# srinix007/GaussianProcessRegression.jl

Hardware: AMD Instinct MI355X
Metric: GP-fit+predict wall-time and K-build GB/s + POTRF TFLOP/s at N=32768 (higher is better)
Workload: dtype f64; 1 GPU; C3 fit+posterior: SE+SE+WN, N=32768, d=8, np=8192; N=32768, d=8, np=8192, kernel=SE+SE+WN, nb=128, parallelism=replicas x1

## Files before the change

### gaussianprocessregression.jl_amd/csrc/common.hpp

```cpp
#pragma once
#include <hip/hip_runtime.h>

#include <cstdio>
#include <string>
#include <vector>

#include "../../include/gpr_hip.h"

#define KMAXP 4

enum { KPROF_SE = 0, KPROF_M32 = 1, KPROF_M52 = 2 };
inline bool kind_stationary(int kind) {
  return kind == GPR_SE || kind == GPR_M32 || kind == GPR_M52 || kind == GPR_PER;
}
inline int kind_hp_width(int kind, int d) {
  return kind == GPR_WN ? 1 : kind == GPR_PER ? 2 * d + 1 : d + 1;
}
inline int kind_profile(int kind) {
  return kind == GPR_M32 ? KPROF_M32 : kind == GPR_M52 ? KPROF_M52 : KPROF_SE;
}
inline const char* kind_name(int kind) {
  return kind == GPR_SE ? "SquaredExp" : kind == GPR_M32 ? "Matern32" : kind == GPR_M52 ? "Matern52"
         : kind == GPR_PER ? "Periodic" : kind == GPR_WN ? "WhiteNoise" : "?";
}

struct KParams {
  int d;
  int nse;
  int has_noise;
  double eps;
  double noise2;
  double noise_sigma;
  double sigma[KMAXP];
  const double* l;
  const double* l2;
  const double* sig;
  const double* pf;
  const double* exptab;
  const int* kinds;
  int nk;
  const double* hp;
  int prof[KMAXP];
  int mix;
  int dx;
  int de;
  int nper;
  const double* per;
  const double* pk;
};

inline KParams kparams_features(const KParams& kp) {
  KParams f = kp;
  f.d = kp.de;
  return f;
}

inline double kp_sigma(const KParams& kp, int p, int* prof = nullptr) {
  int off = 0, se = 0;
  for (int i = 0; i < kp.nk; ++i) {
    if (kp.kinds[i] != GPR_WN) {
      if (se++ == p) {
        if (prof) *prof = kind_profile(kp.kinds[i]);
        return kp.hp[off];
      }
    }
    off += kind_hp_width(kp.kinds[i], kp.dx);
  }
  if (prof) *prof = KPROF_SE;
  return 0.0;
}
inline int kinds_first_non_se(const int* kinds, int nk, int* index) {
  for (int i = 0; i < nk; ++i)
    if (kinds[i] == GPR_M32 || kinds[i] == GPR_M52 || kinds[i] == GPR_PER) {
      if (index) *index = i;
      return kinds[i];
    }
  return 0;
}

inline KParams kparams_group(const KParams& kp, int p0, int cnt, int has_noise) {
  KParams g = kp;
  g.nse = cnt;
  g.has_noise = has_noise;
  g.mix = 0;
  for (int p = 0; p < KMAXP; ++p) {
    g.prof[p] = KPROF_SE;
    g.sigma[p] = p < cnt ? kp_sigma(kp, p0 + p, &g.prof[p]) : 0.0;
    if (g.prof[p] != KPROF_SE) g.mix = 1;
  }
  g.l = kp.l + (size_t)p0 * kp.dx;
  g.l2 = kp.l2 + (size_t)p0 * kp.dx;
  g.sig = kp.sig + p0;
  g.pf = kp.pf + p0;
  if (kp.per) {
    g.per = kp.per + p0;
    g.pk = kp.pk + (size_t)p0 * kp.dx;
  }
  return g;
}

struct KParBlock {
  static constexpr int NSLOT = 8;
  double* dev = nullptr;
  double* host = nullptr;
  size_t cap = 0;
  int next = 0;
  hipEvent_t ev[NSLOT] = {};
  int last = -1;
  size_t last_need = 0;
  int last_nper = 0;
  std::vector<double> tmp;
};

enum TimingClass {
  TC_KBUILD = 0, TC_SYRK = 1, TC_PANEL = 2, TC_TRSM_GEMM = 3, TC_OTHER = 4, TC_GEMM_PIPE = 5,
  TC_DAG = 6, TC_DAG_SOLVE = 7, TC_N = 8
};

struct TimedLaunch {
  int cls;
  hipEvent_t a, b;
  double flops;
};

struct gpr_ctx {
  int device = 0;
  hipStream_t stream = nullptr;
  bool own_stream = false;
  std::string err;
  int nb = 128;
  int nb2 = 1024;
  hipStream_t ls = nullptr;
  hipStream_t stream2 = nullptr;
  hipStream_t srhs = nullptr;
  hipStream_t ssq = nullptr;
  int fused_rhs = -1;
  int fused_rhs_nmax = 16384;
  int fuse_y = 1;
  int fuse_kinv = -1;
  int dag_mode = 1;
  long long dag_spin_limit = 1ll << 25;
  int dag_zlag = 4;
  int dag_lag_built = -1;
  void (*dag_hook)(void* user, const double* dA, int n, int lda, const int* colprog,
                   const int* ustored, int nt, hipEvent_t counters_reset) = nullptr;
  void* dag_hook_user = nullptr;
  int dag_reserve_cu = 0;
  hipEvent_t dag_sync_readers = nullptr;
  bool dag_sync_readers_pending = false;
  bool rhs_solved = false;
  bool gram_full = false;
  int dag_gram = 1;
  int dag_solve = -1;
  int dag_tail = 12288;
  unsigned* dag_tasks = nullptr;
  int dag_ntasks = 0, dag_nt = -1, dag_ntr = -1, dag_flags = -1;
  int* dag_sync = nullptr;
  size_t dag_sync_cap = 0;
  double* dpadA = nullptr;
  size_t padA_cap = 0;
  double* dpadB = nullptr;
  size_t padB_cap = 0;
  void* rb_handle = nullptr;
  int (*rb_destroy)(void*) = nullptr;
  int ncu = 0;
  std::vector<hipEvent_t> sync_events;
  size_t ev_next = 0;

  double* winv = nullptr;
  size_t winv_cap = 0;
  const double* fac_ptr = nullptr;
  int fac_n = 0, fac_ld = 0, fac_nb = 0;
  bool fac_valid = false;

  int* dinfo = nullptr;
  double* dexptab = nullptr;
  double* dscratch = nullptr;
  size_t scratch_cap = 0;
  static constexpr int CV_MAX_SUB = 8;
  struct gpr_ctx* cv_sub[CV_MAX_SUB] = {};
  int cv_streams = 4;
  double* dbig = nullptr;
  size_t big_cap = 0;
  double* dbig2 = nullptr;
  size_t big2_cap = 0;
  double* dsqinv = nullptr;
  size_t sqinv_cap = 0;
  int sqinv_nb2 = 0;
  const double* sq_ptr = nullptr;
  int sq_n = 0, sq_ld = 0;
  double* dpanel = nullptr;
  size_t panel_cap = 0;
  double* dtrsv = nullptr;
  size_t trsv_cap = 0;
  double* dxs = nullptr;
  size_t xs_cap = 0;
  double* dxps = nullptr;
  size_t xps_cap = 0;
  double* dscr_wt = nullptr;
  size_t scr_wt_cap = 0;
  double* dpanel_rhs = nullptr;
  size_t panel_rhs_cap = 0;
  double* dgA = nullptr;
  size_t gA_cap = 0;
  double* dgB = nullptr;
  size_t gB_cap = 0;
  double* dgc = nullptr;
  size_t gc_cap = 0;
  struct KupList {
    long long key = -1;
    int nitems = 0;
    int* d = nullptr;
    unsigned long long used = 0;
  };
  KupList kup[4];
  unsigned long long kup_clock = 0;
  const double* kup_ptr = nullptr;
  int kup_n = 0, kup_ld = 0;
  double* dagb = nullptr;
  size_t dagb_cap = 0;
  double* deig = nullptr;
  size_t eig_cap = 0;
  double* ddc = nullptr;
  size_t dc_cap = 0;
  int* dc_tab_host = nullptr;
  size_t dc_tab_host_cap = 0;
  hipEvent_t dc_tab_ev = nullptr;
  double* dtri = nullptr;
  size_t tri_cap = 0;
  int kbuild_upper = 1;
  int kbuild_exact = 0;
  int kbuild_gram_maxd = 1 << 30;
  KParBlock kpar;
  int kbuild_tiles = 0;
  int kbuild_colstore = 1;
  int cv_batch = 1;
  double cv_batch_gb = 16.0;
  double quad_batch_gb = 16.0;
  int quad_eigen = -1;
  int quad_seq = 0;

  bool timing = false;
  std::vector<TimedLaunch> pending;
  std::vector<hipEvent_t> event_pool;
  double t_ms[TC_N] = {};
  long long t_launches[TC_N] = {};
  double t_flops[TC_N] = {};
};

int split_predict_pieces(gpr_ctx* ctx, const int* kinds, int nk, const double* hp, int d,
                         const double* dX, int ns, const double* dU, int ldu, const double* dwt,
                         const double* dXe, int ne, const double* dXq, int nq, const int* pieces,
                         int npieces, int var_lo, int var_hi, double eps, double* dmu, int ldmu,
                         double* dvar, bool compact);
int set_err(gpr_ctx* ctx, int code, const char* fmt, ...);
void copy_knobs(const gpr_ctx* from, gpr_ctx* to);

#define HIP_TRY(ctx, expr)                                                          \
  do {                                                                              \
    hipError_t _e = (expr);                                                         \
    if (_e != hipSuccess)                                                           \
      return set_err(ctx, GPR_E_HIP, "%s failed: %s (%s:%d)", #expr,                \
                     hipGetErrorString(_e), __FILE__, __LINE__);                    \
  } while (0)

#define GPR_TRY(expr)            \
  do {                           \
    int _r = (expr);             \
    if (_r != 0) return _r;      \
  } while (0)

#define LAUNCH_CHECK(ctx) HIP_TRY(ctx, hipGetLastError())

inline int refuse_non_se(gpr_ctx* ctx, const int* kinds, int nk, const char* what) {
  int idx = 0;
  const int kind = kinds ? kinds_first_non_se(kinds, nk, &idx) : 0;
  if (!kind) return 0;
  return set_err(ctx, GPR_E_UNSUP, "%s needs SquaredExp parts: part %d is %s", what, idx + 1,
                 kind_name(kind));
}

int ensure_buf(gpr_ctx* ctx, double** p, size_t* cap, size_t need_doubles);
int ensure_winv(gpr_ctx* ctx, int n, int nb);

struct TimerScope {
  gpr_ctx* ctx;
  TimedLaunch tl;
  bool on;
  hipStream_t st;
  TimerScope(gpr_ctx* c, int cls, double flops);
  ~TimerScope();
};

int make_kparams(gpr_ctx* ctx, const int* kinds, int nk, const double* hp, int d,
                 double eps, KParams* kp, int* D_total);

// ... 71 lines not shown
```

### gaussianprocessregression.jl_amd/csrc/dag.hip

```cpp
#include <algorithm>
#include <cstdint>
#include <type_traits>

#include "common.hpp"

#ifdef DAG_TRACE
__device__ unsigned long long g_diag_ph[16];
#define DSTAMP_INIT() unsigned long long _dst_t = __builtin_amdgcn_s_memrealtime()
#define DSTAMP(i)                                                   \
  do {                                                              \
    __syncthreads();                                                \
    if (threadIdx.x == 0) {                                         \
      const unsigned long long _t = __builtin_amdgcn_s_memrealtime(); \
      atomicAdd(&g_diag_ph[i], _t - _dst_t);                        \
      if ((i) == 7) atomicAdd(&g_diag_ph[8], 1ull);                 \
      _dst_t = _t;                                                  \
    }                                                               \
  } while (0)
#define DSTAMPW(i)                                                  \
  do {                                                              \
    const unsigned long long _t = __builtin_amdgcn_s_memrealtime(); \
    if (threadIdx.x == 0) atomicAdd(&g_diag_ph[i], _t - _dst_t);    \
    _dst_t = _t;                                                    \
  } while (0)
// ... 441 lines not shown
#pragma unroll
      for (int ii = 0; ii < 4; ++ii)
#pragma unroll
        for (int r = 0; r < 4; ++r) {
          const int nn = wn * 64 + ii * 16 + (lane >> 4) + 4 * r;
          const double* col = T + (size_t)min(nn, nv - 1) * ldt;
#pragma unroll
          for (int jj = 0; jj < 4; ++jj) {
            const int mm = wm * 64 + jj * 16 + (lane & 15);
            const double c = col[min(mm, mv - 1)];
            acc[ii][jj][r] = (mm < mv && nn < nv) ? -c : 0.0;
          }
        }
      if (a.mirror && !rhs && !diag) {
        double* Tm = a.A + (size_t)j * DT + (size_t)i * DT * a.lda;
#pragma unroll
        for (int ii = 0; ii < 4; ++ii)
#pragma unroll
          for (int jj = 0; jj < 4; ++jj)
#pragma unroll
            for (int r = 0; r < 4; ++r) {
              const int nn = wn * 64 + ii * 16 + (lane >> 4) + 4 * r;
              const int mm = wm * 64 + jj * 16 + (lane & 15);
              if (mm < mv && nn < nv) Tm[(size_t)nn + (size_t)mm * a.lda] = -acc[ii][jj][r];
            }
      }
      DTRACE(1, 2);
      int done = (rhs && a.lower) ? j : 0;
      while (done < i) {
        int r = 0;
        PROF(p_wait, r = dag_wait(colprog + i, pj, done, i, a.info, a.spin_limit, &s_wait));
        PROF(p_acc, dag_accum(acc, Pcol + (size_t)done * DT, a.lda, mv, Qcol + (size_t)done * DT,
                              ldt, nv, (r - done) * (DT / DTK), lds));
        done = r;
      }
      if (diag) {
        double* S = lds;
#pragma unroll
        for (int ii = 0; ii < 4; ++ii)
#pragma unroll
          for (int r = 0; r < 4; ++r) {
            const int nn = wn * 64 + ii * 16 + (lane >> 4) + 4 * r;
#pragma unroll
            for (int jj = 0; jj < 4; ++jj) {
              const int mm = wm * 64 + jj * 16 + (lane & 15);
              if (mm <= nn) S[pk(mm, nn)] = nn < mv ? -acc[ii][jj][r] : (mm == nn ? 1.0 : 0.0);
            }
          }
        __syncthreads();
        DTRACE(1, 3);
        int f = 0;
        PROF(p_fac, f = dag_factor(S, mv, a.kglob + i * DT, a.winv + (size_t)i * DT * DT));
        if (f && w == 0) atomicCAS(a.info, 0, f);
        s_fok = f == 0;
        DTRACE(1, 4);
      } else {
        if (i > 0) {
#pragma unroll
          for (int ii = 0; ii < 4; ++ii)
#pragma unroll
            for (int r = 0; r < 4; ++r) {
              const int nn = wn * 64 + ii * 16 + (lane >> 4) + 4 * r;
#pragma unroll
              for (int jj = 0; jj < 4; ++jj) {
                const int mm = wm * 64 + jj * 16 + (lane & 15);
                if (mm < mv && nn < nv) T[(size_t)mm + (size_t)nn * ldt] = -acc[ii][jj][r];
              }
            }
        }
        asm volatile("s_waitcnt vmcnt(0)" ::: "memory");
        __builtin_amdgcn_fence(__ATOMIC_RELEASE, "workgroup");
        PROF(p_wait, dag_wait(colprog + i, colprog + i, i, i + 1, a.info, a.spin_limit, &s_wait));
#pragma unroll
        for (int ii = 0; ii < 4; ++ii)
#pragma unroll
          for (int jj = 0; jj < 4; ++jj) acc[ii][jj] = d4v{0.0, 0.0, 0.0, 0.0};
        const bool tri = mv == DT;
        if (tri)
          PROF(p_tri, dag_accum<true>(acc, a.winv + (size_t)i * DT * DT, DT, mv, T, ldt, nv, DT / DTK, lds));
        else
          PROF(p_tri, dag_accum(acc, a.winv + (size_t)i * DT * DT, DT, mv, T, ldt, nv, mv / DTK, lds));
#pragma unroll
        for (int ii = 0; ii < 4; ++ii)
#pragma unroll
          for (int r = 0; r < 4; ++r) {
            const int nn = wn * 64 + ii * 16 + (lane >> 4) + 4 * r;
#pragma unroll
            for (int jj = 0; jj < 4; ++jj) {
              const int mm = (tri ? 16 * dag_mblk(wm, jj) : wm * 64 + jj * 16) + (lane & 15);
              if (mm < mv && nn < nv) st_res<true>(&T[(size_t)mm + (size_t)nn * ldt], acc[ii][jj][r]);
            }
          }
      }
    } else if (a.mirror && !rhs && !diag) {
      double* Tm = a.A + (size_t)j * DT + (size_t)i * DT * a.lda;
      for (int e = tid; e < DT * DT; e += 256) {
        const int mm = e & (DT - 1), nn = e >> 7;
        if (mm < mv && nn < nv) Tm[(size_t)nn + (size_t)mm * a.lda] = T[(size_t)mm + (size_t)nn * ldt];
      }
    }
    DTRACE(1, 5);
#ifdef DAG_PROF_PUB
    if (diag) PROF(p_pub, dag_publish(pj, i + 1)); else dag_publish(pj, i + 1);
#else
    dag_publish(pj, i + 1);
#endif
    DTRACE(1, 6);
    if (diag && !skip && __builtin_amdgcn_readfirstlane(s_fok))
      dag_store_u(lds, T, a.lda, mv, a.ustored != nullptr);
    if (diag && a.ustored) dag_publish(a.ustored + i, 1);
    ++p_n;
  }
  DTRACE(1, 7);
#ifdef DAG_TRACE
  p_all = __builtin_amdgcn_s_memrealtime() - p_start;
  DTRACE(2, (int)p_wait);
  DTRACE(3, (int)p_acc);
  DTRACE(4, (int)p_fac);
#ifdef DAG_PROF_PUB
#undef p_tri
  DTRACE(5, (int)p_pub);
  (void)p_tri_unused;
#else
  DTRACE(5, (int)p_tri);
#endif
  DTRACE(6, (int)p_all);
  DTRACE(7, (int)p_n);
#endif
}

}

__global__ void dag_init_kernel(int* sync, int nt, int ntr, int solve, int lower) {
  for (int t = blockIdx.x * blockDim.x + threadIdx.x; t < nt + ntr; t += gridDim.x * blockDim.x)
    sync[2 + t] = t < nt ? (solve ? t + 1 : 0) : (lower ? t - nt : 0);
}

static long long dag_spin_limit(const gpr_ctx* ctx) {
#ifdef GPR_TESTING
  if (const char* sl = getenv("GPR_DAG_SPIN_LIMIT")) return std::max(1ll, atoll(sl));
#endif
  return ctx->dag_spin_limit;
}

bool dag_shape_ok(int n, int lda, const double* dA) {
  return n > 0 && n % 16 == 0 && lda % 16 == 0 && lda <= DAG_LD_MAX && ((uintptr_t)dA & 127) == 0 &&
         n <= DT * 32767;
}

extern "C" int gpr_debug_dag_shape_ok(int n, int lda, unsigned long long addr) {
  return dag_shape_ok(n, lda, reinterpret_cast<const double*>((uintptr_t)addr)) ? 1 : 0;
}

bool dag_takes_whole(const gpr_ctx* ctx, int n, int lda, const double* dA) {
  (void)lda;
  (void)dA;
  return ctx->dag_mode && ctx->nb == DT && n > 0 &&
         n <= DT * 32767 - 16;
}

__global__ void dag_pad_in_kernel(const double* __restrict__ A, size_t lda, int n,
                                  double* __restrict__ W, int n2) {
  const size_t tot = (size_t)n2 * n2;
  for (size_t t = blockIdx.x * (size_t)blockDim.x + threadIdx.x; t < tot;
       t += (size_t)gridDim.x * blockDim.x) {
    const int r = (int)(t % n2), c = (int)(t / n2);
    if (r <= c) W[t] = c < n ? A[(size_t)r + (size_t)c * lda] : (r == c ? 1.0 : 0.0);
  }
}

__global__ void dag_pad_out_kernel(double* __restrict__ A, size_t lda, int n,
                                   const double* __restrict__ W, int n2) {
  const size_t tot = (size_t)n * n;
  for (size_t t = blockIdx.x * (size_t)blockDim.x + threadIdx.x; t < tot;
       t += (size_t)gridDim.x * blockDim.x) {
    const int r = (int)(t % n), c = (int)(t / n);
    if (r <= c) A[(size_t)r + (size_t)c * lda] = W[(size_t)r + (size_t)c * n2];
  }
}

int launch_potrf_dag_padded(gpr_ctx* ctx, double* dA, int n, int lda, double* dB, int nrhs,
                            int ldb) {
  const int n2 = (n + 15) / 16 * 16;
  hipStream_t st = ctx->stream;
  if (ensure_buf(ctx, &ctx->dpadA, &ctx->padA_cap, (size_t)n2 * n2) != 0 ||
      (dB && ensure_buf(ctx, &ctx->dpadB, &ctx->padB_cap, (size_t)n2 * nrhs) != 0)) {
    ctx->err.clear();
    (void)hipGetLastError();
    return 1;
  }
  const int blocks = 2048;
  dag_pad_in_kernel<<<blocks, 256, 0, st>>>(dA, (size_t)lda, n, ctx->dpadA, n2);
  LAUNCH_CHECK(ctx);
  if (dB) {
    HIP_TRY(ctx, hipMemcpy2DAsync(ctx->dpadB, (size_t)n2 * sizeof(double), dB,
                                  (size_t)ldb * sizeof(double), (size_t)n * sizeof(double), nrhs,
                                  hipMemcpyDeviceToDevice, st));
    if (n2 > n)
      HIP_TRY(ctx, hipMemset2DAsync(ctx->dpadB + n, (size_t)n2 * sizeof(double), 0,
                                    (size_t)(n2 - n) * sizeof(double), nrhs, st));
  }
  const int rc = launch_potrf_dag(ctx, ctx->dpadA, n2, n2, dB ? ctx->dpadB : nullptr, nrhs, n2, 0,
                                  st, 0);
  if (rc) return rc < 0 ? rc : set_err(ctx, GPR_E_HIP, "padded tile-DAG: shape not eligible");
  dag_pad_out_kernel<<<blocks, 256, 0, st>>>(dA, (size_t)lda, n, ctx->dpadA, n2);
  LAUNCH_CHECK(ctx);
  if (dB)
    HIP_TRY(ctx, hipMemcpy2DAsync(dB, (size_t)ldb * sizeof(double), ctx->dpadB,
                                  (size_t)n2 * sizeof(double), (size_t)n * sizeof(double), nrhs,
                                  hipMemcpyDeviceToDevice, st));
  return 0;
}

int launch_potrf_dag(gpr_ctx* ctx, double* dA, int n, int lda, double* dB, int nrhs, int ldb,
                     int kglob, hipStream_t st, int flags, double* dG, int ldg) {
  const bool solve = flags & DAG_SOLVE, lower = flags & DAG_LOWER, gram = flags & DAG_GRAM;
  const bool mirror = flags & DAG_MIRROR;
  if ((solve || lower) && (!dB || kglob)) return 1;
  if (mirror && (solve || kglob)) return 1;
  if (gram && (!lower || !dG || ldg < n || nrhs != n)) return 1;
  if (ctx->nb != DT || n <= 0 || n % 16 || lda % 16 || lda > DAG_LD_MAX || ((uintptr_t)dA & 127) ||
      n > DT * 32767 || kglob % DT)
    return 1;
  if (dB && (nrhs <= 0 || ldb % 16 || ldb > DAG_LD_MAX || ((uintptr_t)dB & 127) || nrhs > DT * 65535))
    return 1;
  const int nt = (n + DT - 1) / DT, ntr = dB ? (nrhs + DT - 1) / DT : 0;
  GPR_TRY(ensure_winv(ctx, kglob + n, DT));
  if (ctx->dag_nt != nt || ctx->dag_ntr != ntr || ctx->dag_flags != (flags & ~DAG_MIRROR) ||
      ctx->dag_lag_built != ctx->dag_zlag) {
    std::vector<unsigned> tasks;
    tasks.reserve((size_t)nt * (nt + 1) + (size_t)nt * ntr);
    const int lag = solve || !lower ? 0 : std::min(ctx->dag_zlag, nt);
    auto rhs_row = [&](int i) {
      for (int c = 0; c < (lower ? std::min(ntr, i + 1) : ntr); ++c)
        tasks.push_back(0x80000000u | ((unsigned)i << 16) | (unsigned)c);
    };
    for (int i = 0; i < nt; ++i) {
      if (!solve)
        for (int j = i; j < nt; ++j) tasks.push_back(((unsigned)i << 16) | (unsigned)j);
      if (i - lag >= 0) rhs_row(i - lag);
    }
    for (int i = std::max(nt - lag, 0); i < nt; ++i) rhs_row(i);
    if (gram)
      for (int j = 0; j < nt; ++j)
        for (int i = 0; i <= j; ++i) tasks.push_back(((unsigned)i << 16) | (unsigned)j);
    if (ctx->dag_tasks) {
      HIP_TRY(ctx, hipStreamSynchronize(ctx->stream));
      HIP_TRY(ctx, hipFree(ctx->dag_tasks));
    }
    ctx->dag_tasks = nullptr;
    ctx->dag_nt = ctx->dag_ntr = -1;
    HIP_TRY(ctx, hipMalloc((void**)&ctx->dag_tasks, tasks.size() * sizeof(unsigned)));
    HIP_TRY(ctx, hipMemcpy(ctx->dag_tasks, tasks.data(), tasks.size() * sizeof(unsigned),
                           hipMemcpyHostToDevice));
    ctx->dag_ntasks = (int)tasks.size();
    ctx->dag_nt = nt;
    ctx->dag_ntr = ntr;
    ctx->dag_flags = flags & ~DAG_MIRROR;
    ctx->dag_lag_built = ctx->dag_zlag;
  }
  if (ctx->dag_sync_readers_pending) {
    HIP_TRY(ctx, hipStreamWaitEvent(st, ctx->dag_sync_readers, 0));
    HIP_TRY(ctx, hipStreamWaitEvent(ctx->stream, ctx->dag_sync_readers, 0));
    ctx->dag_sync_readers_pending = false;
  }
  const size_t nsync = 2 + (size_t)nt + ntr + nt;
  if (ctx->dag_sync_cap < nsync) {
    if (ctx->dag_sync) {
      HIP_TRY(ctx, hipStreamSynchronize(ctx->stream));
      HIP_TRY(ctx, hipFree(ctx->dag_sync));
    }
    ctx->dag_sync = nullptr;
    ctx->dag_sync_cap = 0;
    HIP_TRY(ctx, hipMalloc((void**)&ctx->dag_sync, nsync * sizeof(int)));
    ctx->dag_sync_cap = nsync;
  }
  HIP_TRY(ctx, hipMemsetAsync(ctx->dag_sync, 0, nsync * sizeof(int), st));
  if (solve || lower) {
    dag_init_kernel<<<(nt + ntr + 255) / 256, 256, 0, st>>>(ctx->dag_sync, nt, ntr, solve, lower);
    LAUNCH_CHECK(ctx);
  }
  if (ctx->ncu <= 0) {
    hipDeviceProp_t prop;
    HIP_TRY(ctx, hipGetDeviceProperties(&prop, ctx->device));
    ctx->ncu = prop.multiProcessorCount;
  }
  DagArgs a{};
  a.A = dA;
  a.lda = (size_t)lda;
  a.n = n;
  a.nt = nt;
  a.B = dB;
  a.ldb = (size_t)(dB ? ldb : 0);
  a.nrhs = dB ? nrhs : 0;
  a.ntr = ntr;
  a.winv = ctx->winv + (size_t)(kglob / DT) * DT * DT;
  a.kglob = kglob;
  a.info = ctx->dinfo;
  a.sync = ctx->dag_sync;
  a.tasks = ctx->dag_tasks;
  a.ntasks = ctx->dag_ntasks;
  a.lower = lower;
  a.G = gram ? dG : nullptr;
  a.ldg = (size_t)(gram ? ldg : 0);
  a.gbase = gram ? ctx->dag_ntasks - nt * (nt + 1) / 2 : ctx->dag_ntasks;
  a.mirror = mirror;
  a.spin_limit = dag_spin_limit(ctx);
  const int grid = std::min(ctx->dag_ntasks, std::max(1, ctx->ncu - ctx->dag_reserve_cu));
  auto hook = (ctx->dag_hook && !solve && !lower && kglob == 0) ? ctx->dag_hook : nullptr;
  a.ustored = hook ? ctx->dag_sync + 2 + nt + ntr : nullptr;
  hipEvent_t hook_ev = nullptr;
  if (hook) {
    ctx->dag_hook = nullptr;
    if (hipEventCreateWithFlags(&hook_ev, hipEventDisableTiming) != hipSuccess) hook_ev = nullptr;
    if (hook_ev && hipEventRecord(hook_ev, st) != hipSuccess) {
      hipEventDestroy(hook_ev);
      hook_ev = nullptr;
    }
    (void)hipGetLastError();
  }
  const double flops = (solve ? 0.0 : (double)n * n * n / 3.0) +
                       (lower ? (double)n * n * n / 3.0 : (double)n * n * (dB ? nrhs : 0)) +
                       (gram ? (double)n * n * n / 3.0 : 0.0);
  {
    hipStream_t ls = ctx->ls;
    ctx->ls = st;
    TimerScope ts(ctx, solve ? TC_DAG_SOLVE : TC_DAG, flops);
    if (gram)
      potrf_dag_kernel<true, false><<<grid, 256, 0, st>>>(a);
    else
      potrf_dag_kernel<false, false><<<grid, 256, 0, st>>>(a);
    ctx->ls = ls;
    const hipError_t le = hipGetLastError();
    if (le != hipSuccess) {
      if (hook_ev) hipEventDestroy(hook_ev);
      return set_err(ctx, GPR_E_HIP, "tile-DAG launch: %s", hipGetErrorString(le));
    }
  }
  if (hook) {
    hook(ctx->dag_hook_user, dA, n, lda, ctx->dag_sync + 2, a.ustored, nt, hook_ev);
    if (hook_ev) hipEventDestroy(hook_ev);
  }
  return 0;
}

int launch_potrf_dag_batch(gpr_ctx* ctx, double* dA, size_t strA, int n, int lda, double* dB,
                           size_t strB, int nrhs, int ldb, int nbatch, int* info_out) {
  hipStream_t st = ctx->stream;
  if (nbatch <= 0) return 0;
  if (n <= 0 || n % 16 || lda % 16 || lda > DAG_LD_MAX || strA % 16 || ((uintptr_t)dA & 127) ||
      n > DT * 32767)
    return 1;
  if (dB && (nrhs <= 0 || ldb % 16 || ldb > DAG_LD_MAX || strB % 16 || ((uintptr_t)dB & 127) ||
             nrhs > DT * 65535))
    return 1;
  const int nt = (n + DT - 1) / DT, ntr = dB ? (nrhs + DT - 1) / DT : 0;
  std::vector<unsigned> tasks;
  std::vector<int> tb;
  const size_t per = (size_t)nt * (nt + 1) / 2 + (size_t)nt * ntr;
  tasks.reserve(per * nbatch);
  tb.reserve(per * nbatch);
  for (int i = 0; i < nt; ++i) {
    for (int b = 0; b < nbatch; ++b)
      for (int j = i; j < nt; ++j) {
        tasks.push_back(((unsigned)i << 16) | (unsigned)j);
        tb.push_back(b);
      }
    for (int b = 0; b < nbatch; ++b)
      for (int c = 0; c < ntr; ++c) {
        tasks.push_back(0x80000000u | ((unsigned)i << 16) | (unsigned)c);
        tb.push_back(b);
      }
  }
  const int ntasks = (int)tasks.size();
  const int strS = 2 + nt + ntr;
  const size_t nW = (size_t)nbatch * nt * DT * DT;
  const size_t nI = (size_t)ntasks * 2 + (size_t)nbatch * strS + (size_t)nbatch;
  GPR_TRY(ensure_buf(ctx, &ctx->dagb, &ctx->dagb_cap, nW + (nI + 1) / 2 + 1));
  double* W = ctx->dagb;
  unsigned* dtasks = reinterpret_cast<unsigned*>(W + nW);
  int* dtb = reinterpret_cast<int*>(dtasks + ntasks);
  int* dsync = dtb + ntasks;
  int* dinfo = dsync + (size_t)nbatch * strS;
  HIP_TRY(ctx, hipMemcpyAsync(dtasks, tasks.data(), sizeof(unsigned) * ntasks, hipMemcpyHostToDevice, st));
  HIP_TRY(ctx, hipMemcpyAsync(dtb, tb.data(), sizeof(int) * ntasks, hipMemcpyHostToDevice, st));
  HIP_TRY(ctx, hipMemsetAsync(dsync, 0, sizeof(int) * ((size_t)nbatch * strS + nbatch), st));
  if (ctx->ncu <= 0) {
    hipDeviceProp_t prop;
    HIP_TRY(ctx, hipGetDeviceProperties(&prop, ctx->device));
    ctx->ncu = prop.multiProcessorCount;
  }
  DagArgs a{};
  a.A = dA;
  a.lda = (size_t)lda;
  a.n = n;
  a.nt = nt;
  a.B = dB;
  a.ldb = (size_t)(dB ? ldb : 0);
  a.nrhs = dB ? nrhs : 0;
  a.ntr = ntr;
  a.winv = W;
  a.kglob = 0;
  a.info = dinfo;
  a.sync = dsync;
  a.tasks = dtasks;
  a.ntasks = ntasks;
  a.gbase = ntasks;
  a.spin_limit = dag_spin_limit(ctx);
  a.tbatch = dtb;
  a.strA = strA;
  a.strB = strB;
  a.strW = (size_t)nt * DT * DT;
// ... 19 lines not shown
```

### gaussianprocessregression.jl_amd/csrc/gpr_ctx.hip

```cpp
#include <algorithm>
#include <cmath>
#include <cstdarg>
#include <cstdlib>
#include <cstring>

#include "common.hpp"

int set_err(gpr_ctx* ctx, int code, const char* fmt, ...) {
  if (ctx) {
    char buf[1024];
    va_list ap;
    va_start(ap, fmt);
    vsnprintf(buf, sizeof buf, fmt, ap);
    va_end(ap);
    ctx->err = buf;
  }
  return code;
}

int ensure_buf(gpr_ctx* ctx, double** p, size_t* cap, size_t need) {
  if (*cap >= need && *p) return 0;
  if (*p) {
    HIP_TRY(ctx, hipStreamSynchronize(ctx->stream));
    HIP_TRY(ctx, hipFree(*p));
// ... 38 lines not shown
TimerScope::~TimerScope() {
  if (!on) return;
  hipEventRecord(tl.b, st);
  ctx->pending.push_back(tl);
}

static void drain_timing(gpr_ctx* ctx) {
  if (ctx->pending.empty()) return;
  hipStreamSynchronize(ctx->stream);
  for (auto& t : ctx->pending) {
    float ms = 0;
    hipEventElapsedTime(&ms, t.a, t.b);
    ctx->t_ms[t.cls] += ms;
    ctx->t_launches[t.cls] += 1;
    ctx->t_flops[t.cls] += t.flops;
    ctx->event_pool.push_back(t.a);
    ctx->event_pool.push_back(t.b);
  }
  ctx->pending.clear();
}

int make_kparams(gpr_ctx* ctx, const int* kinds, int nk, const double* hp, int d, double eps,
                 KParams* kp, int* D_total) {
  if (!kinds || nk <= 0) return set_err(ctx, GPR_E_ARG, "bad kinds/nk (%d)", nk);
  if (!hp) return set_err(ctx, GPR_E_ARG, "hp is NULL");
  if (d <= 0) return set_err(ctx, GPR_E_ARG, "d=%d (needs d >= 1)", d);
  memset(kp, 0, sizeof *kp);
  int nse = 0, nper = 0;
  for (int i = 0, off = 0; i < nk; ++i) {
    if (kind_stationary(kinds[i])) ++nse;
    else if (kinds[i] != GPR_WN) return set_err(ctx, GPR_E_ARG, "unknown kernel kind %d", kinds[i]);
    if (kinds[i] == GPR_PER) {
      ++nper;
      for (int k = 0; k < d; ++k) {
        const double p = hp[off + 1 + d + k];
        if (!(std::fabs(p) > 0.0) || std::isinf(p))
          return set_err(ctx, GPR_E_ARG, "part %d (Periodic): period p_%d = %g of dimension %d is "
                                         "zero or not finite", i + 1, k + 1, p, k + 1);
      }
    }
    off += kind_hp_width(kinds[i], d);
  }
  if (nse == 0)
    return set_err(ctx, GPR_E_ARG, "kernel needs at least one stationary part (SquaredExp, "
                                   "Matern32, Matern52 or Periodic)");
  KParBlock& kb = ctx->kpar;
  const size_t nl = (size_t)nse * d;
  const size_t need = 2 * nl + 2 * (size_t)nse + (nper ? nl + (size_t)nse : 0);
  if (need > kb.cap || !kb.dev) {
    const size_t cap = std::max(need, (size_t)(2 * 4 * 64 + 2 * 4));
    if (kb.dev) {
      HIP_TRY(ctx, hipStreamSynchronize(ctx->stream));
      HIP_TRY(ctx, hipFree(kb.dev));
      HIP_TRY(ctx, hipHostFree(kb.host));
      kb.dev = kb.host = nullptr;
      kb.cap = 0;
    }
    const size_t bytes = KParBlock::NSLOT * cap * sizeof(double);
    if (hipMalloc((void**)&kb.dev, bytes) != hipSuccess) {
      kb.dev = nullptr;
      return set_err(ctx, GPR_E_NOMEM, "hipMalloc of %zu bytes failed", bytes);
    }
    if (hipHostMalloc((void**)&kb.host, bytes, hipHostMallocDefault) != hipSuccess) {
      hipFree(kb.dev);
      kb.dev = kb.host = nullptr;
      return set_err(ctx, GPR_E_NOMEM, "hipHostMalloc of %zu bytes failed", bytes);
    }
    kb.cap = cap;
    kb.last = -1;
  }
  kb.tmp.resize(need);
  double* hl = kb.tmp.data();
  kp->exptab = ctx->dexptab;
  kp->d = kp->dx = d;
  kp->de = nper ? 2 * d : d;
  kp->nper = nper;
  kp->eps = eps;
  kp->kinds = kinds;
  kp->nk = nk;
  kp->hp = hp;
  int off = 0;
  for (int i = 0; i < nk; ++i) {
    if (kinds[i] != GPR_WN) {
      const int prof = kind_profile(kinds[i]);
      if (kp->nse < KMAXP) {
        kp->sigma[kp->nse] = hp[off];
        kp->prof[kp->nse] = prof;
      }
      if (prof != KPROF_SE) kp->mix = 1;
      hl[2 * nl + kp->nse] = hp[off];
      hl[2 * nl + nse + kp->nse] = (double)prof;
      for (int k = 0; k < d; ++k) {
        hl[(size_t)kp->nse * d + k] = hp[off + 1 + k];
        hl[nl + (size_t)kp->nse * d + k] = hp[off + 1 + k] * hp[off + 1 + k];
      }
      if (nper) {
        const bool per = kinds[i] == GPR_PER;
        hl[2 * nl + 2 * nse + kp->nse] = per ? 1.0 : 0.0;
        for (int k = 0; k < d; ++k)
          hl[2 * nl + 3 * (size_t)nse + (size_t)kp->nse * d + k] = per ? hp[off + 1 + d + k] : 1.0;
      }
      kp->nse++;
      off += kind_hp_width(kinds[i], d);
    } else {
      if (!kp->has_noise) {
        kp->has_noise = 1;
        kp->noise_sigma = hp[off];
        kp->noise2 = hp[off] * hp[off];
      }
      off += 1;
    }
  }
  int slot = kb.last;
  if (slot < 0 || kb.last_need != need || kb.last_nper != nper ||
      memcmp(kb.host + (size_t)slot * kb.cap, hl, need * sizeof(double)) != 0) {
    slot = kb.next;
    kb.next = (slot + 1) % KParBlock::NSLOT;
    if (!kb.ev[slot]) HIP_TRY(ctx, hipEventCreateWithFlags(&kb.ev[slot], hipEventDisableTiming));
    else HIP_TRY(ctx, hipEventSynchronize(kb.ev[slot]));
    kb.last = -1;
    memcpy(kb.host + (size_t)slot * kb.cap, hl, need * sizeof(double));
    HIP_TRY(ctx, hipMemcpyAsync(kb.dev + (size_t)slot * kb.cap, kb.host + (size_t)slot * kb.cap,
                                need * sizeof(double), hipMemcpyHostToDevice, ctx->stream));
    HIP_TRY(ctx, hipEventRecord(kb.ev[slot], ctx->stream));
    kb.last = slot;
    kb.last_need = need;
    kb.last_nper = nper;
  }
  const double* dl = kb.dev + (size_t)slot * kb.cap;
  kp->l = dl;
  kp->l2 = dl + nl;
  kp->sig = dl + 2 * nl;
  kp->pf = dl + 2 * nl + nse;
  if (nper) {
    kp->per = dl + 2 * nl + 2 * nse;
    kp->pk = dl + 2 * nl + 3 * (size_t)nse;
  }
  if (D_total) *D_total = off;
  return 0;
}

namespace {
struct Knob {
  const char* name;
  int gpr_ctx::*ip;
  double gpr_ctx::*dp;
};
const Knob kKnobs[] = {
    {"GPR_DAG", &gpr_ctx::dag_mode, nullptr},
    {"GPR_DAG_TAIL", &gpr_ctx::dag_tail, nullptr},
    {"GPR_DAG_SOLVE", &gpr_ctx::dag_solve, nullptr},
    {"GPR_DAG_GRAM", &gpr_ctx::dag_gram, nullptr},
    {"GPR_DAG_ZLAG", &gpr_ctx::dag_zlag, nullptr},
    {"GPR_FUSED_RHS", &gpr_ctx::fused_rhs, nullptr},
    {"GPR_FUSE_Y", &gpr_ctx::fuse_y, nullptr},
    {"GPR_FUSE_KINV", &gpr_ctx::fuse_kinv, nullptr},
    {"GPR_KBUILD_UPPER", &gpr_ctx::kbuild_upper, nullptr},
    {"GPR_KBUILD_EXACT", &gpr_ctx::kbuild_exact, nullptr},
    {"GPR_KBUILD_COLSTORE", &gpr_ctx::kbuild_colstore, nullptr},
    {"GPR_KBUILD_TILES", &gpr_ctx::kbuild_tiles, nullptr},
    {"GPR_KBUILD_GRAM_MAXD", &gpr_ctx::kbuild_gram_maxd, nullptr},
    {"GPR_CV_STREAMS", &gpr_ctx::cv_streams, nullptr},
    {"GPR_CV_BATCH", &gpr_ctx::cv_batch, nullptr},
    {"GPR_CV_BATCH_GB", nullptr, &gpr_ctx::cv_batch_gb},
    {"GPR_QUAD_BATCH_GB", nullptr, &gpr_ctx::quad_batch_gb},
    {"GPR_QUAD_EIGEN", &gpr_ctx::quad_eigen, nullptr},
    {"GPR_QUAD_SEQ", &gpr_ctx::quad_seq, nullptr},
};

void knob_set(gpr_ctx* ctx, const Knob& k, double v) {
  if (k.ip) {
    int iv = (int)v;
    if (k.ip == &gpr_ctx::dag_zlag) iv = std::max(0, iv);
    if (k.ip == &gpr_ctx::cv_streams) iv = std::max(1, std::min(iv, (int)gpr_ctx::CV_MAX_SUB));
    ctx->*k.ip = iv;
  } else {
    ctx->*k.dp = v;
  }
}

const Knob* knob_find(const char* name) {
  if (!name) return nullptr;
  for (const Knob& k : kKnobs)
    if (!strcmp(k.name, name)) return &k;
  return nullptr;
}
}

void copy_knobs(const gpr_ctx* from, gpr_ctx* to) {
  for (const Knob& k : kKnobs) {
    if (k.ip) to->*k.ip = from->*k.ip;
    else to->*k.dp = from->*k.dp;
  }
  to->dag_spin_limit = from->dag_spin_limit;
}

extern "C" {

const char* gpr_version(void) { return "gpr_hip 0.1.0 (gfx950)"; }

int gpr_ctx_create(int device, void* stream, gpr_ctx_t* out) {
  if (!out) return GPR_E_ARG;
  *out = nullptr;
  gpr_ctx* ctx = new gpr_ctx();
  ctx->device = device;
  if (hipSetDevice(device) != hipSuccess) {
    delete ctx;
    return GPR_E_HIP;
  }
  if (stream) {
    ctx->stream = (hipStream_t)stream;
  } else {
    if (hipStreamCreateWithFlags(&ctx->stream, hipStreamNonBlocking) != hipSuccess) {
      delete ctx;
      return GPR_E_HIP;
    }
    ctx->own_stream = true;
  }
  ctx->ls = ctx->stream;
  int prio_lo = 0, prio_hi = 0;
  hipDeviceGetStreamPriorityRange(&prio_lo, &prio_hi);
  if (hipStreamCreateWithPriority(&ctx->stream2, hipStreamNonBlocking, prio_hi) != hipSuccess ||
      hipStreamCreateWithFlags(&ctx->srhs, hipStreamNonBlocking) != hipSuccess ||
      hipStreamCreateWithFlags(&ctx->ssq, hipStreamNonBlocking) != hipSuccess) {
    delete ctx;
    return GPR_E_HIP;
  }
  if (const char* e = getenv("GPU_MAX_HW_QUEUES")) {
    const int q = atoi(e);
    if (q > 0) ctx->cv_streams = std::min(ctx->cv_streams, q);
  }
  for (const Knob& k : kKnobs)
    if (const char* e = getenv(k.name)) knob_set(ctx, k, atof(e));
  if (hipMalloc((void**)&ctx->dinfo, 64) != hipSuccess) {
    delete ctx;
    return GPR_E_NOMEM;
  }
  {
    double tab[256];
    for (int j = 0; j < 256; ++j) tab[j] = (double)exp2l((long double)j / 256.0L);
    if (hipMalloc((void**)&ctx->dexptab, sizeof tab) != hipSuccess ||
        hipMemcpy(ctx->dexptab, tab, sizeof tab, hipMemcpyHostToDevice) != hipSuccess) {
      hipFree(ctx->dinfo);
      delete ctx;
      return GPR_E_NOMEM;
    }
  }
  *out = ctx;
  return 0;
}

int gpr_ctx_destroy(gpr_ctx_t ctx) {
  if (!ctx) return 0;
  for (auto* sub : ctx->cv_sub) gpr_ctx_destroy(sub);
  hipStreamSynchronize(ctx->stream);
  if (ctx->dag_sync_readers) {
    hipEventSynchronize(ctx->dag_sync_readers);
    hipEventDestroy(ctx->dag_sync_readers);
  }
  drain_timing(ctx);
  for (auto e : ctx->event_pool) hipEventDestroy(e);
  for (auto e : ctx->sync_events) hipEventDestroy(e);
  if (ctx->stream2) hipStreamDestroy(ctx->stream2);
  if (ctx->srhs) hipStreamDestroy(ctx->srhs);
  if (ctx->ssq) hipStreamDestroy(ctx->ssq);
  if (ctx->dpanel_rhs) hipFree(ctx->dpanel_rhs);
  if (ctx->dscr_wt) hipFree(ctx->dscr_wt);
  if (ctx->dag_tasks) hipFree(ctx->dag_tasks);
  if (ctx->dag_sync) hipFree(ctx->dag_sync);
  if (ctx->dpadA) hipFree(ctx->dpadA);
  if (ctx->dpadB) hipFree(ctx->dpadB);
  if (ctx->rb_handle && ctx->rb_destroy) ctx->rb_destroy(ctx->rb_handle);
  if (ctx->winv) hipFree(ctx->winv);
  if (ctx->dinfo) hipFree(ctx->dinfo);
  if (ctx->dexptab) hipFree(ctx->dexptab);
  if (ctx->dscratch) hipFree(ctx->dscratch);
  if (ctx->dbig) hipFree(ctx->dbig);
  if (ctx->dbig2) hipFree(ctx->dbig2);
  if (ctx->dtrsv) hipFree(ctx->dtrsv);
  if (ctx->dsqinv) hipFree(ctx->dsqinv);
  if (ctx->dpanel) hipFree(ctx->dpanel);
  if (ctx->dxs) hipFree(ctx->dxs);
  if (ctx->dxps) hipFree(ctx->dxps);
  if (ctx->dgA) hipFree(ctx->dgA);
  if (ctx->dgB) hipFree(ctx->dgB);
  if (ctx->dgc) hipFree(ctx->dgc);
  if (ctx->kpar.dev) hipFree(ctx->kpar.dev);
  if (ctx->kpar.host) hipHostFree(ctx->kpar.host);
  for (auto e : ctx->kpar.ev)
    if (e) hipEventDestroy(e);
  for (auto& e : ctx->kup)
    if (e.d) hipFree(e.d);
  if (ctx->deig) hipFree(ctx->deig);
  if (ctx->ddc) hipFree(ctx->ddc);
  if (ctx->dc_tab_ev) hipEventDestroy(ctx->dc_tab_ev);
  if (ctx->dc_tab_host) hipHostFree(ctx->dc_tab_host);
  if (ctx->dtri) hipFree(ctx->dtri);
  if (ctx->dagb) hipFree(ctx->dagb);
  if (ctx->own_stream) hipStreamDestroy(ctx->stream);
  delete ctx;
  return 0;
}

const char* gpr_last_error(gpr_ctx_t ctx) { return ctx ? ctx->err.c_str() : "null context"; }

int gpr_sync(gpr_ctx_t ctx) {
  HIP_TRY(ctx, hipStreamSynchronize(ctx->stream));
  return 0;
}

void* gpr_ctx_stream(gpr_ctx_t ctx) { return ctx ? (void*)ctx->stream : nullptr; }

int gpr_malloc(gpr_ctx_t ctx, size_t bytes, void** dptr) {
  if (!dptr) return set_err(ctx, GPR_E_ARG, "dptr is NULL");
  if (hipMalloc(dptr, bytes ? bytes : 1) != hipSuccess)
    return set_err(ctx, GPR_E_NOMEM, "hipMalloc(%zu) failed", bytes);
  return 0;
}

int gpr_free(gpr_ctx_t ctx, void* dptr) {
  HIP_TRY(ctx, hipStreamSynchronize(ctx->stream));
  if (dptr) HIP_TRY(ctx, hipFree(dptr));
  return 0;
}

int gpr_upload(gpr_ctx_t ctx, void* dst, const void* src, size_t bytes) {
  HIP_TRY(ctx, hipMemcpyAsync(dst, src, bytes, hipMemcpyHostToDevice, ctx->stream));
  HIP_TRY(ctx, hipStreamSynchronize(ctx->stream));
  return 0;
}

int gpr_download(gpr_ctx_t ctx, void* dst, const void* src, size_t bytes) {
  HIP_TRY(ctx, hipMemcpyAsync(dst, src, bytes, hipMemcpyDeviceToHost, ctx->stream));
  HIP_TRY(ctx, hipStreamSynchronize(ctx->stream));
  return 0;
}

int gpr_set_block(gpr_ctx_t ctx, int nb) {
  if (nb != 64 && nb != 128) return set_err(ctx, GPR_E_ARG, "nb must be 64 or 128 (got %d)", nb);
  ctx->nb = nb;
  if (ctx->nb2 % nb) ctx->nb2 = 4 * nb;
  ctx->fac_valid = false;
  return 0;
}

int gpr_set_outer_block(gpr_ctx_t ctx, int nb2) {
  if (nb2 < ctx->nb || nb2 % ctx->nb)
    return set_err(ctx, GPR_E_ARG, "outer block %d must be a multiple of nb=%d", nb2, ctx->nb);
  ctx->nb2 = nb2;
  return 0;
}

int gpr_set_knob(gpr_ctx_t ctx, const char* name, double value) {
  if (!ctx) return GPR_E_ARG;
  const Knob* k = knob_find(name);
  if (!k) return set_err(ctx, GPR_E_ARG, "unknown knob %s", name ? name : "(null)");
  knob_set(ctx, *k, value);
  if (k->ip == &gpr_ctx::dag_zlag) ctx->dag_lag_built = -1;
  return 0;
}

int gpr_get_knob(gpr_ctx_t ctx, const char* name, double* value) {
  if (!ctx || !value) return GPR_E_ARG;
  const Knob* k = knob_find(name);
  if (!k) return set_err(ctx, GPR_E_ARG, "unknown knob %s", name ? name : "(null)");
  *value = k->ip ? (double)(ctx->*k->ip) : ctx->*k->dp;
  return 0;
}

int gpr_forget_factor(gpr_ctx_t ctx) {
  ctx->fac_valid = false;
  ctx->fac_ptr = nullptr;
  ctx->sqinv_nb2 = 0;
  ctx->sq_ptr = nullptr;
  return 0;
}

int gpr_timing_enable(gpr_ctx_t ctx, int on) {
  ctx->timing = on != 0;
  return 0;
}

int gpr_timing_get(gpr_ctx_t ctx, int cls, double* ms, long long* launches, double* flops) {
  if (cls < 0 || cls >= TC_N) return set_err(ctx, GPR_E_ARG, "bad timing class %d", cls);
  drain_timing(ctx);
  if (ms) *ms = ctx->t_ms[cls];
  if (launches) *launches = ctx->t_launches[cls];
  if (flops) *flops = ctx->t_flops[cls];
  return 0;
}

int gpr_timing_reset(gpr_ctx_t ctx) {
  drain_timing(ctx);
  for (int i = 0; i < TC_N; ++i) {
    ctx->t_ms[i] = 0;
    ctx->t_launches[i] = 0;
    ctx->t_flops[i] = 0;
  }
  return 0;
}

}
```

Before: 3.380 GP jobs/s (fit N=32768 + posterior mean/var np=8192, per GPU).

## Interleave DAG task order across row groups after a leading panel

Adds a configurable task ordering for the persistent DAG Cholesky/solve scheduler. For non-lower, non-gram runs, rows past a threshold (default 32) are emitted in groups of up to 4 and interleaved column by column, optionally with a skew between rows. The aim is to expose more concurrent ready tasks and reduce stalls waiting on dependencies late in the factorization. The interleaving can also delay the critical-path panel tasks. Knobs and a debug export are added, and the rebuild key now covers the new parameters.

```diff
diff --git a/gaussianprocessregression.jl_amd/csrc/common.hpp b/gaussianprocessregression.jl_amd/csrc/common.hpp
--- a/gaussianprocessregression.jl_amd/csrc/common.hpp
+++ b/gaussianprocessregression.jl_amd/csrc/common.hpp
@@ -141,7 +141,8 @@
   int dag_mode = 1;
   long long dag_spin_limit = 1ll << 25;
   int dag_zlag = 4;
-  int dag_lag_built = -1;
+  int dag_rgroup = 4, dag_rskew = 0, dag_rgroup_min = 32;
+  int dag_order_built[4] = {-1, -1, -1, -1};
   void (*dag_hook)(void* user, const double* dA, int n, int lda, const int* colprog,
                    const int* ustored, int nt, hipEvent_t counters_reset) = nullptr;
   void* dag_hook_user = nullptr;
diff --git a/gaussianprocessregression.jl_amd/csrc/dag.hip b/gaussianprocessregression.jl_amd/csrc/dag.hip
--- a/gaussianprocessregression.jl_amd/csrc/dag.hip
+++ b/gaussianprocessregression.jl_amd/csrc/dag.hip
@@ -617,6 +617,56 @@
   return dag_shape_ok(n, lda, reinterpret_cast<const double*>((uintptr_t)addr)) ? 1 : 0;
 }
 
+std::vector<unsigned> dag_task_order(int nt, int ntr, bool solve, bool lower, bool gram, int zlag,
+                                     int group, int skew, int gmin) {
+  std::vector<unsigned> tasks;
+  tasks.reserve((size_t)nt * (nt + 1) + (size_t)nt * ntr);
+  const int lag = solve || !lower ? 0 : std::min(std::max(zlag, 0), nt);
+  auto a_task = [&](int i, int j) { tasks.push_back(((unsigned)i << 16) | (unsigned)j); };
+  auto rhs_task = [&](int i, int c) {
+    tasks.push_back(0x80000000u | ((unsigned)i << 16) | (unsigned)c);
+  };
+  auto rhs_row = [&](int i) {
+    for (int c = 0; c < (lower ? std::min(ntr, i + 1) : ntr); ++c) rhs_task(i, c);
+  };
+  const int R = (lower || gram || group < 2) ? 1 : (group < 4 ? 2 : 4);
+  const int g0 = R == 1 ? nt : (int)std::min<long long>(nt, ((long long)std::max(gmin, 0) + R - 1) / R * R);
+  const int sk = std::min(std::max(skew, 0), std::max(nt, ntr));
+  for (int i = 0; i < g0; ++i) {
+    if (!solve)
+      for (int j = i; j < nt; ++j) a_task(i, j);
+    if (i - lag >= 0) rhs_row(i - lag);
+  }
+  for (int i = std::max(nt - lag, 0); i < nt; ++i) rhs_row(i);
+  for (int g = g0; g < nt; g += R) {
+    const int m = std::min(R, nt - g);
+    if (!solve)
+      for (int s = 0; s < nt - g + (m - 1) * sk; ++s)
+        for (int r = 0; r < m; ++r) {
+          const int j = g + s - r * sk;
+          if (j >= g + r && j < nt) a_task(g + r, j);
+        }
+    for (int s = 0; s < ntr + (m - 1) * sk; ++s)
+      for (int r = 0; r < m; ++r) {
+        const int c = s - r * sk;
+        if (c >= 0 && c < ntr) rhs_task(g + r, c);
+      }
+  }
+  if (gram)
+    for (int j = 0; j < nt; ++j)
+      for (int i = 0; i <= j; ++i) a_task(i, j);
+  return tasks;
+}
+
+extern "C" int gpr_debug_dag_task_order(int nt, int ntr, int flags, int zlag, int group, int skew,
+                                        int gmin, unsigned* out, int cap) {
+  if (nt <= 0 || nt > 32767 || ntr < 0 || ntr > 65535) return -1;
+  const std::vector<unsigned> t = dag_task_order(nt, ntr, flags & DAG_SOLVE, flags & DAG_LOWER,
+                                                 flags & DAG_GRAM, zlag, group, skew, gmin);
+  for (size_t k = 0; k < t.size() && (long long)k < cap; ++k) out[k] = t[k];
+  return (int)t.size();
+}
+
 bool dag_takes_whole(const gpr_ctx* ctx, int n, int lda, const double* dA) {
   (void)lda;
   (void)dA;
@@ -691,24 +741,11 @@
     return 1;
   const int nt = (n + DT - 1) / DT, ntr = dB ? (nrhs + DT - 1) / DT : 0;
   GPR_TRY(ensure_winv(ctx, kglob + n, DT));
+  const int key[4] = {ctx->dag_zlag, ctx->dag_rgroup, ctx->dag_rskew, ctx->dag_rgroup_min};
   if (ctx->dag_nt != nt || ctx->dag_ntr != ntr || ctx->dag_flags != (flags & ~DAG_MIRROR) ||
-      ctx->dag_lag_built != ctx->dag_zlag) {
-    std::vector<unsigned> tasks;
-    tasks.reserve((size_t)nt * (nt + 1) + (size_t)nt * ntr);
-    const int lag = solve || !lower ? 0 : std::min(ctx->dag_zlag, nt);
-    auto rhs_row = [&](int i) {
-      for (int c = 0; c < (lower ? std::min(ntr, i + 1) : ntr); ++c)
-        tasks.push_back(0x80000000u | ((unsigned)i << 16) | (unsigned)c);
-    };
-    for (int i = 0; i < nt; ++i) {
-      if (!solve)
-        for (int j = i; j < nt; ++j) tasks.push_back(((unsigned)i << 16) | (unsigned)j);
-      if (i - lag >= 0) rhs_row(i - lag);
-    }
-    for (int i = std::max(nt - lag, 0); i < nt; ++i) rhs_row(i);
-    if (gram)
-      for (int j = 0; j < nt; ++j)
-        for (int i = 0; i <= j; ++i) tasks.push_back(((unsigned)i << 16) | (unsigned)j);
+      !std::equal(key, key + 4, ctx->dag_order_built)) {
+    const std::vector<unsigned> tasks =
+        dag_task_order(nt, ntr, solve, lower, gram, key[0], key[1], key[2], key[3]);
     if (ctx->dag_tasks) {
       HIP_TRY(ctx, hipStreamSynchronize(ctx->stream));
       HIP_TRY(ctx, hipFree(ctx->dag_tasks));
@@ -722,7 +759,7 @@
     ctx->dag_nt = nt;
     ctx->dag_ntr = ntr;
     ctx->dag_flags = flags & ~DAG_MIRROR;
-    ctx->dag_lag_built = ctx->dag_zlag;
+    std::copy(key, key + 4, ctx->dag_order_built);
   }
   if (ctx->dag_sync_readers_pending) {
     HIP_TRY(ctx, hipStreamWaitEvent(st, ctx->dag_sync_readers, 0));
diff --git a/gaussianprocessregression.jl_amd/csrc/gpr_ctx.hip b/gaussianprocessregression.jl_amd/csrc/gpr_ctx.hip
--- a/gaussianprocessregression.jl_amd/csrc/gpr_ctx.hip
+++ b/gaussianprocessregression.jl_amd/csrc/gpr_ctx.hip
@@ -214,6 +214,9 @@
     {"GPR_DAG_SOLVE", &gpr_ctx::dag_solve, nullptr},
     {"GPR_DAG_GRAM", &gpr_ctx::dag_gram, nullptr},
     {"GPR_DAG_ZLAG", &gpr_ctx::dag_zlag, nullptr},
+    {"GPR_DAG_RGROUP", &gpr_ctx::dag_rgroup, nullptr},
+    {"GPR_DAG_RSKEW", &gpr_ctx::dag_rskew, nullptr},
+    {"GPR_DAG_RGROUP_MIN", &gpr_ctx::dag_rgroup_min, nullptr},
     {"GPR_FUSED_RHS", &gpr_ctx::fused_rhs, nullptr},
     {"GPR_FUSE_Y", &gpr_ctx::fuse_y, nullptr},
     {"GPR_FUSE_KINV", &gpr_ctx::fuse_kinv, nullptr},
@@ -234,6 +237,8 @@
   if (k.ip) {
     int iv = (int)v;
     if (k.ip == &gpr_ctx::dag_zlag) iv = std::max(0, iv);
+    if (k.ip == &gpr_ctx::dag_rgroup) iv = iv < 2 ? 1 : (iv < 4 ? 2 : 4);
+    if (k.ip == &gpr_ctx::dag_rskew || k.ip == &gpr_ctx::dag_rgroup_min) iv = std::max(0, iv);
     if (k.ip == &gpr_ctx::cv_streams) iv = std::max(1, std::min(iv, (int)gpr_ctx::CV_MAX_SUB));
     ctx->*k.ip = iv;
   } else {
@@ -418,7 +423,6 @@
   const Knob* k = knob_find(name);
   if (!k) return set_err(ctx, GPR_E_ARG, "unknown knob %s", name ? name : "(null)");
   knob_set(ctx, *k, value);
-  if (k->ip == &gpr_ctx::dag_zlag) ctx->dag_lag_built = -1;
   return 0;
 }
 
```

Result: faster. 3.464 GP jobs/s (fit N=32768 + posterior mean/var np=8192, per GPU), median of 6 (+2.5%).
